# ArmingLou/seed-vc

Hardware: AMD Instinct MI355X
Metric: mel_frames_per_sec (higher is better)
Workload: dtype f16; 1 GPU; seed-uvit-tat-xlsr-tiny CFM 25 steps cfg 0.7 + HiFT, batch 64 x (P=430,S=430) per GPU; batch_per_gpu=64, global_batch=64, prompt_frames=430, diffusion_steps=25, vocoder_precision=fp16p8, lanes_per_gpu=2, parallelism=utterance-sharded x1, audio gather on rank 0

## Files before the change

seed-vc_amd/csrc/common.h:

```cpp
#pragma once
#include <atomic>
#include <hip/hip_runtime.h>
#include <stdint.h>
#include <stdio.h>
#include <string>

namespace svc {

typedef _Float16 half_t;
typedef _Float16 half8 __attribute__((ext_vector_type(8)));
typedef _Float16 half4 __attribute__((ext_vector_type(4)));
typedef _Float16 half2v __attribute__((ext_vector_type(2)));
typedef float float4v __attribute__((ext_vector_type(4)));
typedef unsigned int u32x4 __attribute__((ext_vector_type(4)));

void set_error(const std::string& msg);
const char* get_error();

#define SVC_CHECK_HIP(expr)                                                                  \
    do {                                                                                     \
        hipError_t _e = (expr);                                                              \
        if (_e != hipSuccess) {                                                              \
            svc::set_error(std::string(#expr) + ": " + hipGetErrorString(_e) + " at " + __FILE__ + \
                           ":" + std::to_string(__LINE__));                                  \
            return 1;                                                                        \
        }                                                                                    \
    } while (0)

#define SVC_REQUIRE(cond, msg)                                                               \
    do {                                                                                     \
        if (!(cond)) {                                                                       \
            svc::set_error(std::string("requirement failed: ") + #cond + " -- " + (msg));    \
            return 1;                                                                        \
        }                                                                                    \
    } while (0)

__device__ __forceinline__ float sin_sq(float x) {
    const float n = rintf(x * 0.318309886183790672f);
    float r = fmaf(n, -3.140625f, x);
    r = fmaf(n, -9.67502593994140625e-4f, r);
    r = fmaf(n, -1.509957990978376e-7f, r);
    const float r2 = r * r;
    float p = fmaf(r2, 2.6348154733568663e-06f, -0.00019822761532850564f);
    p = fmaf(p, r2, 0.008333242498338223f);
    p = fmaf(p, r2, -0.1666666567325592f);
    const float sn = fmaf(p * r2, r, r);
    return sn * sn;
}

struct DeviceState {
    int device = -1;
    void* zero_page = nullptr;
    std::atomic<unsigned long long> kconv_attr{0};
    std::atomic<bool> fused_attr{false};
};
DeviceState* device_state();
int current_device();

enum { PROF_KGEMM_F16 = 0, PROF_KGEMM_F32 = 1, PROF_ATTN = 2, PROF_FUSED = 3, PROF_N = 4 };
bool prof_enabled();
void prof_begin(int cls, hipStream_t st);
void prof_end(int cls, double flops, double bytes, hipStream_t st, unsigned long long tag = 0);

template <int MAXA, int DPT>
__device__ __forceinline__ void wait_tiles(int ahead) {
    static_assert(MAXA * DPT <= 63, "vmcnt is a 6-bit counter");
    if constexpr (MAXA <= 0) {
        asm volatile("s_waitcnt vmcnt(0)" ::: "memory");
    } else {
        if (ahead >= MAXA) asm volatile("s_waitcnt vmcnt(%0)" ::"n"(MAXA * DPT) : "memory");
        else wait_tiles<MAXA - 1, DPT>(ahead);
    }
}

__device__ __forceinline__ float act_apply(float v, int act, float slope);
__device__ __forceinline__ uint4 pack8(const float* v) {
    half8 h;
#pragma unroll
    for (int j = 0; j < 8; ++j) h[j] = (half_t)v[j];
    return *reinterpret_cast<uint4*>(&h);
}

static inline int cdiv(long a, long b) { return (int)((a + b - 1) / b); }
static inline long round_up(long a, long b) { return (a + b - 1) / b * b; }

constexpr int KG_MAX_TAPS = 48;

enum { KG_PAD_ZERO = 0, KG_PAD_REFLECT = 1, KG_PAD_CLAMP = 2 };
enum { KG_ACT_NONE = 0, KG_ACT_SILU = 1, KG_ACT_ELU = 2, KG_ACT_LRELU = 3, KG_ACT_TANH = 4, KG_ACT_ABS = 5,
       KG_ACT_CLAMP = 6 , KG_ACT_SIGMOID = 7,
       KG_ACT_GELU = 8  };
enum {
    KG_EPI_STORE = 0,
    KG_EPI_SWIGLU = 1,
    KG_EPI_TANHSIG = 2,
    KG_EPI_QKV_ROPE = 3,
    KG_EPI_STORE_GELU = 4,
};

__device__ __forceinline__ float gelu_erf(float v) { return 0.5f * v * (1.0f + erff(v * 0.70710678118654752f)); }

__device__ __forceinline__ float act_apply(float v, int act, float slope) {
    switch (act) {
        case KG_ACT_SILU: return v / (1.0f + __expf(-v));
        case KG_ACT_ELU: return v > 0.f ? v : (expm1f(v));
        case KG_ACT_LRELU: return v > 0.f ? v : v * slope;
        case KG_ACT_TANH: return tanhf(v);
        case KG_ACT_ABS: return fabsf(v);
        case KG_ACT_CLAMP: return fminf(fmaxf(v, -slope), slope);
        case KG_ACT_SIGMOID: return 1.0f / (1.0f + __expf(-v));
        default: return v;
    }
}

struct KGemmParams {
    const void* a_ptr[KG_MAX_TAPS];
    long a_ld[KG_MAX_TAPS];
    int a_shift[KG_MAX_TAPS];
    int a_ktiles[KG_MAX_TAPS];
    int n_taps;
    int Lout, a_seq_rows, a_off, a_stride, a_len, pad_mode;
    int reflect_min;
    const int* seq_len;
    const void* zero_page;
    float prof_flop_scale;
    int debug;
    int group_n;
    const void* w;
    long ldw;
    int M, N;
    int c_seq_rows, c_off;
    float* c32; long ldc32;
    half_t* c16; long ldc16;
    const float* post_a; const float* post_ib; int post_n; half_t* c16_lo;
    const float* bias;
    const float* rowvec; long ld_rowvec;
    const float* gate;   long ld_gate;
    const float* res;    long ldres;
    const float* res2;   long ldres2;
    float out_scale;
    int act; float act_slope;
    int post_relu;
    int vec_ok;
    const float* rope;
    int rope_D;
    float q_scale;
    half_t* vt; long vt_seq_stride; long vt_ld;
    int vt_mode;
};

int kgemm_launch(const KGemmParams& p, int dtype , int epi, hipStream_t st);
int kgemm_big_launch(const KGemmParams& p, int epi, hipStream_t st);

struct KConvParams {
    const void* a_hi; const void* a_lo;
// ... 87 lines not shown
```

seed-vc_amd/csrc/conv_util.h:

```cpp
#pragma once
#include <stdlib.h>
#include <string.h>

#include <string>

#include "model_util.h"

namespace svc {

struct ConvW {
    void* w = nullptr;
    float* bias = nullptr;
    long ldw = 0;
    int k = 0, cin_pad = 0, cout = 0, cout_pad = 0, dtype = 0, vd = 0;
    void* w8 = nullptr;
    long ldw8 = 0;
    int w8_exp = 0;
    int stride = 0;
};

inline int gdt(int vd) { return vd == 1 ? 1 : 0; }
inline bool is_split(int vd) { return vd == 2 || vd == 3; }
inline int cpad(int c, int vd) { return (int)round_up(c, ktile_elems(gdt(vd))); }
inline size_t vesize(int vd) { return esize(gdt(vd)); }
// ... 92 lines not shown
                } else {
                    if (pack_f16_launch(ws.v + kk, reinterpret_cast<half_t*>(out->w) + off, cin, cout, 1, (long)cout * k, k, 0, 1,
                                        out->ldw, 0, ws.scale, st)) return 1;
                }
            }
        }
        SVC_CHECK_HIP(hipMemcpyAsync(out->bias + (long)r * out->cout_pad, b->data, cout * sizeof(float),
                                     hipMemcpyDeviceToDevice, st));
    }
    return 0;
}

struct ConvRun {
    ActBuf a;
    int B = 0, Lin = 0, Lout = 0;
    int dilation = 1, stride = 1, pad_left = 0, pad_mode = KG_PAD_ZERO;
    float* c32 = nullptr; long ldc32 = 0;
    half_t* c16 = nullptr; long ldc16 = 0;
    int c_rows = 0, c_off = 0;
    const float* res = nullptr; long ldres = 0;
    const float* res2 = nullptr; long ldres2 = 0;
    float out_scale = 0.f;
    int act = KG_ACT_NONE; float act_slope = 0.f;
    int n_override = 0;
    const int* seq_len = nullptr;
    bool seq_kconv = false;
    const float* post_a = nullptr; const float* post_ib = nullptr; int post_n = 0; half_t* c16_lo = nullptr;
    int c16_lo_fmt = 0;
    bool p8 = false;
    int bm = 0;
    bool force_gemm = false;
    int* took = nullptr;
};

inline int kconv_min_n() {
    static const int v = [] { const char* e = getenv("SVC_KCONV_MIN_N"); return e ? atoi(e) : 64; }();
    return v;
}

constexpr int KCONV_MIN_ROWS = 192;

inline bool conv_p8_ok(const ConvW& w, int Lout, int dilation) {
    return w.w8 != nullptr && kconv_enabled() && (w.k - 1) * dilation <= 64 && Lout >= KCONV_MIN_ROWS && w.cout_pad >= kconv_min_n() &&
           w.cout_pad % 8 == 0;
}

inline int conv1d_run(const ConvW& w, const ConvRun& r, hipStream_t st) {
    KGemmParams p;
    memset(&p, 0, sizeof(p));
    const int nsub = is_split(w.vd) ? 3 : 1;
    SVC_REQUIRE(w.k * nsub <= KG_MAX_TAPS, "conv kernel size exceeds the tap limit");
    p.M = r.B * r.Lout;
    p.N = r.n_override ? r.n_override : w.cout_pad;
    p.Lout = r.Lout;
    p.a_seq_rows = r.Lin;
    p.a_len = r.Lin;
    p.seq_len = r.seq_len;
    p.a_stride = r.stride;
    p.pad_mode = r.pad_mode;
    p.n_taps = w.k * nsub;
    const int kt = w.cin_pad / ktile_elems(w.dtype);
    for (int t = 0; t < w.k; ++t)
        for (int sub = 0; sub < nsub; ++sub) {
            const int i = t * nsub + sub;
            p.a_ptr[i] = sub == 2 ? r.a.lo : r.a.hi;
            p.a_ld[i] = w.cin_pad;
            p.a_ktiles[i] = kt;
            p.a_shift[i] = t * r.dilation - r.pad_left;
        }
    p.w = w.w;
    p.ldw = w.ldw;
    p.bias = w.bias;
    p.c_seq_rows = r.c_rows ? r.c_rows : r.Lout;
    p.c_off = r.c_off;
    p.c32 = r.c32; p.ldc32 = r.ldc32;
    p.c16 = r.c16; p.ldc16 = r.ldc16;
    p.res = r.res; p.ldres = r.ldres;
    p.res2 = r.res2; p.ldres2 = r.ldres2;
    p.out_scale = r.out_scale;
    p.act = r.act; p.act_slope = r.act_slope;
    p.post_a = r.post_a; p.post_ib = r.post_ib; p.post_n = r.post_n; p.c16_lo = r.c16_lo;
    p.prof_flop_scale = 1.0f / nsub;
    p.vec_ok = (p.N % 8 == 0) && (r.ldc32 % 8 == 0) && (r.ldc16 % 8 == 0) && (r.ldres % 8 == 0) && (r.ldres2 % 8 == 0);
    const bool kconv_ok = !r.force_gemm && kconv_enabled() && w.dtype == 0 && r.stride == 1 && w.k >= 3 && (w.k - 1) * r.dilation <= 64 &&
                          r.pad_mode == KG_PAD_ZERO && (!r.seq_len || (r.seq_kconv && r.Lin == r.Lout)) && !r.n_override && p.vec_ok &&
                          r.Lout >= KCONV_MIN_ROWS && w.cin_pad >= 64 &&
                          p.N >= kconv_min_n();
    SVC_REQUIRE((!r.p8 && !r.c16_lo_fmt) || (kconv_ok && (!r.p8 || conv_p8_ok(w, r.Lout, r.dilation))),
                "conv1d_run: the fp8-pair operand format needs the resident-tile kernel");
    if (kconv_ok) {
        KConvParams q;
        memset(&q, 0, sizeof(q));
        q.a_hi = r.a.hi; q.a_lo = r.a.lo; q.w = r.p8 ? w.w8 : w.w; q.ldw = r.p8 ? w.ldw8 : w.ldw; q.bias = w.bias;
        q.B = r.B; q.Lin = r.Lin; q.Lout = r.Lout; q.N = p.N; q.cin_pad = w.cin_pad; q.k = w.k; q.dil = r.dilation;
        q.pad_left = r.pad_left; q.nsub = r.p8 ? 2 : nsub; q.w8_exp = w.w8_exp; q.c16_lo_fmt = r.c16_lo_fmt;
        q.c_seq_rows = p.c_seq_rows; q.c_off = p.c_off;
        q.c32 = r.c32; q.ldc32 = r.ldc32; q.c16 = r.c16; q.c16_lo = r.c16_lo; q.ldc16 = r.ldc16;
        q.post_a = r.post_a; q.post_ib = r.post_ib; q.post_n = r.post_n;
        q.res = r.res; q.ldres = r.ldres; q.res2 = r.res2; q.ldres2 = r.ldres2;
        q.out_scale = r.out_scale; q.act = r.act; q.act_slope = r.act_slope;
        q.seq_len = r.seq_len;
        q.bm = r.bm; q.took = r.took;
        return kconv_launch(q, st);
    }
    if (r.took) *r.took = 0;
    return kgemm_launch(p, w.dtype, KG_EPI_STORE, st);
}

inline int convT_run(const ConvW& w, ActBuf a, int B, int L, float* c32, int c_rows_q, int c_off_q, hipStream_t st,
                     const int* seq_len = nullptr) {
    KGemmParams p;
    memset(&p, 0, sizeof(p));
    const int nsub = is_split(w.vd) ? 3 : 1;
    p.M = B * L;
    p.N = w.stride * w.cout_pad;
    p.Lout = L;
    p.a_seq_rows = L;
    p.a_len = L;
    p.seq_len = seq_len;
    p.a_stride = 1;
    p.pad_mode = KG_PAD_ZERO;
    p.n_taps = 3 * nsub;
    const int kt = w.cin_pad / ktile_elems(w.dtype);
    for (int t = 0; t < 3; ++t)
        for (int sub = 0; sub < nsub; ++sub) {
            const int i = t * nsub + sub;
            p.a_ptr[i] = sub == 2 ? a.lo : a.hi;
            p.a_ld[i] = w.cin_pad;
            p.a_ktiles[i] = kt;
            p.a_shift[i] = t - 1;
        }
    p.w = w.w;
    p.ldw = w.ldw;
    p.bias = w.bias;
    p.c_seq_rows = c_rows_q ? c_rows_q : L;
    p.c_off = c_off_q;
    p.c32 = c32;
    p.ldc32 = p.N;
    p.vec_ok = 1;
    p.prof_flop_scale = 1.0f / nsub;
    return kgemm_launch(p, w.dtype, KG_EPI_STORE, st);
}

}
```

seed-vc_amd/csrc/fused.hip:

```cpp
#include <stdlib.h>

#include <utility>

#include "common.h"

namespace svc {

namespace {

typedef __attribute__((address_space(1))) const void* gptr_t;
typedef __attribute__((address_space(3))) void* lptr_t;

template <int D>
struct PG {
    static constexpr int NT = D / 16;
    static constexpr int KC = D / 32;
    static constexpr int SLOT_BYTES = NT * 1024;
    static constexpr int NS = D == 384 ? 5 : 4;
    static constexpr int RING = NS * SLOT_BYTES;
    static constexpr int PF = D == 384 ? 6 : 4;
    static constexpr int NVEC = 9;
    static constexpr int LDS = RING + NVEC * D * 4;
};

__device__ __forceinline__ half8 frag_read(unsigned lds_addr, int off) {
    half8 r;
    asm volatile("ds_read_b128 %0, %1 offset:%2" : "=v"(r) : "v"(lds_addr), "n"(0) : "memory");
    (void)off;
    return r;
}
template <int OFF>
__device__ __forceinline__ void frag_read_to(half8& r, unsigned lds_addr) {
    asm volatile("ds_read_b128 %0, %1 offset:%2" : "=v"(r) : "v"(lds_addr), "n"(OFF));
}
template <int N>
__device__ __forceinline__ void frag_wait(half8& r) {
    asm volatile("s_waitcnt lgkmcnt(%1)" : "+v"(r) : "n"(N));
}

template <int NF, int PF, int TM, int RFI, typename F, typename R>
__device__ __forceinline__ void stream_frags(const char* base, F&& body, R&& refill) {
    static_assert(NF * 1024 <= 65536 && PF >= 1 && PF <= 8, "ds_read offset field");
    const unsigned la = (unsigned)(uintptr_t)(lptr_t)const_cast<char*>(base);
    half8 q[PF];
    [&]<int... I>(std::integer_sequence<int, I...>) { (frag_read_to<I * 1024>(q[I], la), ...); }(std::make_integer_sequence<int, PF>{});
    [&]<int... Fi>(std::integer_sequence<int, Fi...>) {
        ([&] {
            constexpr int f = Fi;
            constexpr int pending = (NF - f < PF ? NF - f : PF) - 1;
            frag_wait<pending>(q[f % PF]);
            const half8 w = q[f % PF];
            body(f, w);
            if constexpr (f + PF < NF) frag_read_to<(f + PF) * 1024>(q[f % PF], la);
            if constexpr (f % RFI == RFI - 1) refill(f / RFI);
            __builtin_amdgcn_sched_barrier(0);
        }(), ...);
    }(std::make_integer_sequence<int, NF>{});
}

__device__ __forceinline__ void mfma_v(float4v& c, const half8 a, const half8 b) {
    asm volatile("v_mfma_f32_16x16x32_f16 %0, %1, %2, %0" : "+v"(c) : "v"(a), "v"(b));
}
__device__ __forceinline__ void mfma_guard(float4v (&a)[4][2]) {
    asm volatile("s_nop 15\n\ts_nop 3"
                 : "+v"(a[0][0]), "+v"(a[0][1]), "+v"(a[1][0]), "+v"(a[1][1]), "+v"(a[2][0]), "+v"(a[2][1]), "+v"(a[3][0]), "+v"(a[3][1]));
}
__device__ __forceinline__ void mfma_guard(float4v (&a)[4][1]) {}
template <int NF, typename F, typename R>
__device__ __forceinline__ void stream_frags_asm(const char* base, F&& body, R&& refill) {
    static_assert(NF % 4 == 0, "fragment groups of 4");
    half8 q[2][4];
#pragma unroll
    for (int i = 0; i < 4; ++i) q[0][i] = *reinterpret_cast<const half8*>(base + i * 1024);
#pragma unroll
    for (int g = 0; g < NF / 4; ++g) {
        if (g + 1 < NF / 4) {
#pragma unroll
            for (int i = 0; i < 4; ++i) q[(g + 1) & 1][i] = *reinterpret_cast<const half8*>(base + ((g + 1) * 4 + i) * 1024);
        }
        __builtin_amdgcn_sched_barrier(0);
#pragma unroll
        for (int i = 0; i < 4; ++i) body(g * 4 + i, q[g & 1][i]);
        refill(g);
        __builtin_amdgcn_sched_barrier(0);
    }
}

enum { V_AF = 0, V_BF = 1, V_GA = 2, V_GF = 3, V_AA = 4, V_BA = 5, V_BS = 6, V_AN = 7, V_BN = 8 };

template <int D, bool GATED, int TM>
__global__ __launch_bounds__(128 / (16 * TM) * 64, 128 / (16 * TM) / 4) void dit_panel_kernel(const PanelParams p) {
    using G = PG<D>;
    constexpr int NT = G::NT, KC = G::KC, NS = G::NS, PF = G::PF;
    constexpr int NW = 128 / (16 * TM), NTHR = NW * 64, DPS = NT / NW, RFI = NT / DPS;
    constexpr bool ASM_SIDE = D == 512 && TM == 2;
    extern __shared__ __attribute__((aligned(16))) char smem[];
    float* vec = reinterpret_cast<float*>(smem + G::RING);

    const int tid = threadIdx.x, lane = tid & 63;
    const int wave = __builtin_amdgcn_readfirstlane(tid >> 6);
    const int fr = lane & 15, fq = lane >> 4;
    const int m0 = blockIdx.x * 128 + wave * (16 * TM);

    for (int c = tid; c < D; c += NTHR) {
        const float one = p.add_one ? 1.f : 0.f;
        vec[V_AF * D + c] = p.g_ffn ? p.g_ffn[c] * (p.w_f ? one + p.w_f[c] : 1.f) : 0.f;
        vec[V_BF * D + c] = p.b_f ? p.b_f[c] : 0.f;
        vec[V_GA * D + c] = p.gate_a ? p.gate_a[c] : 1.f;
        vec[V_GF * D + c] = p.gate_f ? p.gate_f[c] : 1.f;
        vec[V_AA * D + c] = p.g_attn ? p.g_attn[c] * (p.w_a ? one + p.w_a[c] : 1.f) : 0.f;
        vec[V_BA * D + c] = p.b_a ? p.b_a[c] : 0.f;
        vec[V_BS * D + c] = p.bskip ? p.bskip[c] : 0.f;
        vec[V_AN * D + c] = p.g_fin ? p.g_fin[c] * (p.w_fin ? one + p.w_fin[c] : 1.f) : 0.f;
        vec[V_BN * D + c] = p.b_fin ? p.b_fin[c] : 0.f;
    }
    __syncthreads();

    const char* wsrc = reinterpret_cast<const char*>(p.wstream) + wave * (G::SLOT_BYTES / NW) + lane * 16;
    int s_next = 0, stage = 0, fill = NS - 1, s_issued = 0;
    auto piece = [&](const char* src, char* dst, int i) {
// ... 508 lines not shown
```

seed-vc_amd/csrc/kconv.hip:

```cpp
#include <math.h>
#include <stdlib.h>
#include <string.h>

#include "common.h"

namespace svc {

namespace {

constexpr int CB_NW = 8, CB_NT = CB_NW * 64;
constexpr int CB_SPAN = 64;
constexpr int cb_a_bytes(int bm) { return (bm + CB_SPAN) * 128; }
constexpr int CB_EPI_LD = 68;
constexpr int cb_ns(int bn, int bm) { return bm == 128 ? 2 : (bm < 256 ? 3 : (bn == 128 ? 5 : 8)); }
constexpr int cb_lds(int bn, int bm) { return 2 * cb_a_bytes(bm) + cb_ns(bn, bm) * bn * 128; }

__device__ __forceinline__ int cswz(int row) { return row & 7; }

template <int NSUB, int BN, int BM, bool RAGGED>
__global__ __launch_bounds__(CB_NT, BM < 256 ? 2 : 1) void kconv_kernel(const KConvParams p) {
    constexpr int CB_N = BN, CB_M = BM;
    constexpr int CB_NS = cb_ns(BN, BM);
    constexpr int CB_A_BYTES = cb_a_bytes(BM);
    constexpr int CB_W_BYTES = BN * 128;
    constexpr int WROWS_M = BN == 128 ? BM / 4 : BM / 8;
    constexpr int TM = WROWS_M / 16;
    static_assert(TM >= 1, "tile");
    constexpr int WDPT = BN / 64;
    extern __shared__ __attribute__((aligned(16))) char smem[];
    char* a_hi = smem;
    char* a_lo = smem + CB_A_BYTES;
    char* w_ring = smem + 2 * CB_A_BYTES;

    const int tid = threadIdx.x, lane = tid & 63, wave = tid >> 6;
    const int wave_u = __builtin_amdgcn_readfirstlane(wave);
    const int n_mt = (p.Lout + CB_M - 1) / CB_M;
    const int n_nt = (p.N + CB_N - 1) / CB_N;
    const int nblk = gridDim.x;
    const int xq = nblk >> 3, xr = nblk & 7, xcd = blockIdx.x & 7;
    const int bid = (xcd < xr ? xcd * (xq + 1) : xr * (xq + 1) + (xcd - xr) * xq) + (blockIdx.x >> 3);
    const int tile_n = bid % n_nt;
    const int rest = bid / n_nt;
    const int tile_m = rest % n_mt;
    const int b = rest / n_mt;
    const int p0 = tile_m * CB_M;
    int lin = p.Lin;
    if constexpr (RAGGED) {
        lin = p.seq_len[b];
        if (p0 >= lin) return;
    }
    const int n0 = tile_n * CB_N;
    const int span = (p.k - 1) * p.dil;
    const int R = CB_M + span;
    const int nchunks = p.cin_pad / 64;
    const int total = nchunks * p.k * NSUB;

    typedef __attribute__((address_space(1))) const void* gptr_t;
    typedef __attribute__((address_space(3))) void* lptr_t;
    const char* zero_ = reinterpret_cast<const char*>(p.zero_page);

    const int wm0 = BN == 128 ? (wave >> 1) * WROWS_M : wave * WROWS_M, wn0 = BN == 128 ? (wave & 1) * 64 : 0;
    const int fr = lane & 15, fq = lane >> 4;
    float4v acc[TM][4];
#pragma unroll
    for (int i = 0; i < TM; ++i)
#pragma unroll
        for (int j = 0; j < 4; ++j) acc[i][j] = (float4v){0.f, 0.f, 0.f, 0.f};

    const int c8 = tid & 7, rr = tid >> 3;
    const half_t* wrow[WDPT];
#pragma unroll
    for (int i = 0; i < WDPT; ++i) {
        const int row = rr + 64 * i;
        wrow[i] = reinterpret_cast<const half_t*>(p.w) + (long)(n0 + row) * p.ldw + ((c8 ^ cswz(row)) << 3);
    }
    auto issue_w = [&](int it, int stage) {
        const int c = it / (p.k * NSUB);
        const int ts = it - c * (p.k * NSUB);
        const long col = (long)ts * p.cin_pad + 64L * c;
        char* dst = w_ring + stage * CB_W_BYTES + wave_u * 1024;
#pragma unroll
        for (int i = 0; i < WDPT; ++i)
            __builtin_amdgcn_global_load_lds((gptr_t)(wrow[i] + col), (lptr_t)(dst + i * 64 * 128), 16, 0, 0);
    };
    auto issue_a = [&](int c) {
        for (int i = 0; i * 64 < R; ++i) {
            const int row = rr + 64 * i;
            const int pos = p0 - p.pad_left + row;
            const bool ok = (row < R) & (pos >= 0) & (pos < lin);
            const long off = (((long)b * p.Lin + (ok ? pos : 0)) * p.cin_pad + 64L * c + ((c8 ^ cswz(row)) << 3)) * 2;
            const char* sh = ok ? reinterpret_cast<const char*>(p.a_hi) + off : zero_;
            __builtin_amdgcn_global_load_lds((gptr_t)sh, (lptr_t)(a_hi + (64 * i + wave_u * 8) * 128), 16, 0, 0);
            if constexpr (NSUB != 1) {
                const char* sl = ok ? reinterpret_cast<const char*>(p.a_lo) + off : zero_;
                __builtin_amdgcn_global_load_lds((gptr_t)sl, (lptr_t)(a_lo + (64 * i + wave_u * 8) * 128), 16, 0, 0);
            }
        }
    };

#pragma unroll
    for (int s_ = 0; s_ < CB_NS - 1; ++s_)
        if (s_ < total) issue_w(s_, s_);
    int stage = 0, fill = CB_NS - 1, it = 0;
    for (int c = 0; c < nchunks; ++c) {
        asm volatile("s_waitcnt vmcnt(0)" ::: "memory");
        asm volatile("s_barrier" ::: "memory");
        issue_a(c);
        asm volatile("s_waitcnt vmcnt(0)" ::: "memory");
        asm volatile("s_barrier" ::: "memory");
        for (int t = 0; t < p.k; ++t) {
            const int shift = t * p.dil;
#pragma unroll
            for (int s = 0; s < NSUB; ++s, ++it) {
                const int ahead = total - 1 - it;
                wait_tiles<CB_NS - 2, WDPT>(ahead);
                asm volatile("s_barrier" ::: "memory");
                if (it + CB_NS - 1 < total) issue_w(it + CB_NS - 1, fill);
                const char* at = ((NSUB == 3 && s == 2) || (NSUB == 2 && s == 1)) ? a_lo : a_hi;
                const char* wt = w_ring + stage * CB_W_BYTES;
                if constexpr (NSUB == 2) {
                    if (s == 1) {
                        typedef int v8i __attribute__((ext_vector_type(8)));
                        v8i af8[TM], bf8[4];
#pragma unroll
                        for (int mt = 0; mt < TM; ++mt) {
                            const int row = wm0 + mt * 16 + fr + shift;
                            const u32x4 x0 = *reinterpret_cast<const u32x4*>(at + row * 128 + ((fq ^ cswz(row)) << 4));
                            const u32x4 x1 = *reinterpret_cast<const u32x4*>(at + row * 128 + (((4 + fq) ^ cswz(row)) << 4));
                            af8[mt] = (v8i){(int)x0[0], (int)x0[1], (int)x0[2], (int)x0[3], (int)x1[0], (int)x1[1], (int)x1[2], (int)x1[3]};
                        }
#pragma unroll
                        for (int nt = 0; nt < 4; ++nt) {
                            const int row = wn0 + nt * 16 + fr;
                            const u32x4 x0 = *reinterpret_cast<const u32x4*>(wt + row * 128 + ((fq ^ cswz(row)) << 4));
                            const u32x4 x1 = *reinterpret_cast<const u32x4*>(wt + row * 128 + (((4 + fq) ^ cswz(row)) << 4));
                            bf8[nt] = (v8i){(int)x0[0], (int)x0[1], (int)x0[2], (int)x0[3], (int)x1[0], (int)x1[1], (int)x1[2], (int)x1[3]};
                        }
                        const int sc_a = 127 - 11, sc_b = 127 - p.w8_exp;
#pragma unroll
                        for (int mt = 0; mt < TM; ++mt)
#pragma unroll
                            for (int nt = 0; nt < 4; ++nt)
                                acc[mt][nt] = __builtin_amdgcn_mfma_scale_f32_16x16x128_f8f6f4(af8[mt], bf8[nt], acc[mt][nt], 0, 0, 0, sc_a, 0, sc_b);
                        stage = stage + 1 == CB_NS ? 0 : stage + 1;
                        fill = fill + 1 == CB_NS ? 0 : fill + 1;
                        continue;
                    }
                }
#pragma unroll
                for (int ks = 0; ks < 2; ++ks) {
                    u32x4 af[TM], bf[4];
                    const int chunk = ks * 4 + fq;
#pragma unroll
                    for (int mt = 0; mt < TM; ++mt) {
                        const int row = wm0 + mt * 16 + fr + shift;
                        af[mt] = *reinterpret_cast<const u32x4*>(at + row * 128 + ((chunk ^ cswz(row)) << 4));
                    }
#pragma unroll
                    for (int nt = 0; nt < 4; ++nt) {
                        const int row = wn0 + nt * 16 + fr;
                        bf[nt] = *reinterpret_cast<const u32x4*>(wt + row * 128 + ((chunk ^ cswz(row)) << 4));
                    }
#pragma unroll
                    for (int mt = 0; mt < TM; ++mt)
#pragma unroll
                        for (int nt = 0; nt < 4; ++nt)
                            acc[mt][nt] = __builtin_amdgcn_mfma_f32_16x16x32_f16(__builtin_bit_cast(half8, af[mt]),
                                                                                 __builtin_bit_cast(half8, bf[nt]), acc[mt][nt], 0, 0, 0);
                }
                stage = stage + 1 == CB_NS ? 0 : stage + 1;
                fill = fill + 1 == CB_NS ? 0 : fill + 1;
            }
        }
    }
    asm volatile("s_waitcnt vmcnt(0)" ::: "memory");
    __syncthreads();

    constexpr int RP = TM >= 2 ? 32 : 16;
    float* ep = reinterpret_cast<float*>(smem) + wave * RP * CB_EPI_LD;
#pragma unroll
    for (int pass = 0; pass < TM * 16 / RP; ++pass) {
        if (pass > 0) __syncthreads();
#pragma unroll
        for (int mi = 0; mi < RP / 16; ++mi)
#pragma unroll
            for (int nt = 0; nt < 4; ++nt)
#pragma unroll
                for (int r = 0; r < 4; ++r)
                    ep[(mi * 16 + fq * 4 + r) * CB_EPI_LD + nt * 16 + fr] = acc[pass * (RP / 16) + mi][nt][r];
        __syncthreads();
#pragma unroll
        for (int i = 0; i < RP / 8; ++i) {
            const int ch = lane + 64 * i;
            const int row = ch >> 3, cc = ch & 7;
            const int pos = p0 + wm0 + pass * RP + row;
            const int n = n0 + wn0 + cc * 8;
            float v[8];
            {
                const float4v x0 = *reinterpret_cast<const float4v*>(ep + row * CB_EPI_LD + cc * 8);
                const float4v x1 = *reinterpret_cast<const float4v*>(ep + row * CB_EPI_LD + cc * 8 + 4);
#pragma unroll
                for (int j = 0; j < 4; ++j) { v[j] = x0[j]; v[4 + j] = x1[j]; }
            }
            if (pos >= p.Lout || n >= p.N) continue;
            const long orow = (long)b * p.c_seq_rows + p.c_off + pos;
            if (p.bias) {
                const float4v b0 = *reinterpret_cast<const float4v*>(p.bias + n);
                const float4v b1 = *reinterpret_cast<const float4v*>(p.bias + n + 4);
#pragma unroll
                for (int j = 0; j < 4; ++j) { v[j] += b0[j]; v[4 + j] += b1[j]; }
            }
            if (p.act != KG_ACT_NONE) {
#pragma unroll
                for (int j = 0; j < 8; ++j) v[j] = act_apply(v[j], p.act, p.act_slope);
            }
            if (p.res) {
                const float4v q0 = *reinterpret_cast<const float4v*>(p.res + orow * p.ldres + n);
                const float4v q1 = *reinterpret_cast<const float4v*>(p.res + orow * p.ldres + n + 4);
#pragma unroll
                for (int j = 0; j < 4; ++j) { v[j] += q0[j]; v[4 + j] += q1[j]; }
            }
            if (p.out_scale != 0.f) {
#pragma unroll
                for (int j = 0; j < 8; ++j) v[j] *= p.out_scale;
            }
            if (p.res2) {
                const float4v q0 = *reinterpret_cast<const float4v*>(p.res2 + orow * p.ldres2 + n);
                const float4v q1 = *reinterpret_cast<const float4v*>(p.res2 + orow * p.ldres2 + n + 4);
#pragma unroll
                for (int j = 0; j < 4; ++j) { v[j] += q0[j]; v[4 + j] += q1[j]; }
            }
            if (p.c32) {
                *reinterpret_cast<float4v*>(p.c32 + orow * p.ldc32 + n) = (float4v){v[0], v[1], v[2], v[3]};
                *reinterpret_cast<float4v*>(p.c32 + orow * p.ldc32 + n + 4) = (float4v){v[4], v[5], v[6], v[7]};
            }
            if (p.post_a) {
                float lo[8];
                float hf[8];
#pragma unroll
                for (int j = 0; j < 8; ++j) {
                    const int nn = n + j;
                    const float sv = nn < p.post_n ? v[j] + p.post_ib[nn] * sin_sq(p.post_a[nn] * v[j]) : 0.f;
                    const half_t hh = (half_t)sv;
                    v[j] = sv;
                    lo[j] = sv - (float)hh;
                    hf[j] = (float)hh;
                }
                if (p.c16_lo) {
                    if (p.c16_lo_fmt) {
                                const u32x4 pr = {lo_pair_p8(hf[0], lo[0]) | (lo_pair_p8(hf[1], lo[1]) << 16), lo_pair_p8(hf[2], lo[2]) | (lo_pair_p8(hf[3], lo[3]) << 16),
                                                  lo_pair_p8(hf[4], lo[4]) | (lo_pair_p8(hf[5], lo[5]) << 16), lo_pair_p8(hf[6], lo[6]) | (lo_pair_p8(hf[7], lo[7]) << 16)};
                                *reinterpret_cast<u32x4*>(p.c16_lo + orow * p.ldc16 + n) = pr;
                            }
                    else *reinterpret_cast<uint4*>(p.c16_lo + orow * p.ldc16 + n) = pack8(lo);
                }
            }
            if (p.c16) *reinterpret_cast<uint4*>(p.c16 + orow * p.ldc16 + n) = pack8(v);
        }
    }
}


__global__ void absmax_kernel(const float* __restrict__ src, int n0, int n1, int n2, long s0, long s1, long s2,
                              const float* __restrict__ scale, float* __restrict__ out) {
    __shared__ float red[256];
    float m = 0.f;
    const long total = (long)n0 * n1 * n2;
    for (long i = (long)blockIdx.x * 256 + threadIdx.x; i < total; i += 256L * gridDim.x) {
        const int i2 = (int)(i % n2);
        const long r = i / n2;
        const int i1 = (int)(r % n1), i0 = (int)(r / n1);
        float v = src[i0 * s0 + i1 * s1 + i2 * s2];
        if (scale) v *= scale[i0];
        m = fmaxf(m, fabsf(v));
    }
    red[threadIdx.x] = m;
    __syncthreads();
    for (int o = 128; o > 0; o >>= 1) {
        if ((int)threadIdx.x < o) red[threadIdx.x] = fmaxf(red[threadIdx.x], red[threadIdx.x + o]);
        __syncthreads();
    }
    if (threadIdx.x == 0) atomicMax(reinterpret_cast<unsigned*>(out), __float_as_uint(red[0]));
}

__global__ void pack_p8_kernel(const float* __restrict__ src, unsigned short* __restrict__ dst, int n0, int n1, int n2, long s0, long s1,
                               long s2, long d0, long d1, long d2, const float* __restrict__ scale, float sw) {
    const long i = (long)blockIdx.x * blockDim.x + threadIdx.x;
    const long total = (long)n0 * n1 * n2;
    if (i >= total) return;
    const int i2 = (int)(i % n2);
    const long r = i / n2;
    const int i1 = (int)(r % n1), i0 = (int)(r / n1);
    float v = src[i0 * s0 + i1 * s1 + i2 * s2];
    if (scale) v *= scale[i0];
    const float hi = (float)(half_t)v, lo = v - hi;
    const float b0 = fminf(fmaxf(lo * sw * 2048.f, -448.f), 448.f), b1 = fminf(fmaxf(hi * sw, -448.f), 448.f);
    dst[i0 * d0 + i1 * d1 + i2 * d2] = (unsigned short)((unsigned)__builtin_amdgcn_cvt_pk_fp8_f32(b0, b1, 0, false) & 0xffffu);
}

}

int kconv_pack_p8(const float* src, unsigned short* dst, int n0, int n1, int n2, long s0, long s1, long s2, long d0, long d1, long d2,
                  const float* scale, int* exp_out, hipStream_t st) {
    float* d_max = nullptr;
    SVC_CHECK_HIP(hipMalloc(&d_max, sizeof(float)));
    SVC_CHECK_HIP(hipMemsetAsync(d_max, 0, sizeof(float), st));
    hipLaunchKernelGGL(absmax_kernel, dim3(256), dim3(256), 0, st, src, n0, n1, n2, s0, s1, s2, scale, d_max);
    float mx = 0.f;
    hipError_t e = hipMemcpyAsync(&mx, d_max, sizeof(float), hipMemcpyDeviceToHost, st);
    if (e == hipSuccess) e = hipStreamSynchronize(st);
    (void)hipFree(d_max);
    SVC_CHECK_HIP(e);
    int ex = 0;
    if (mx > 0.f) {
        ex = (int)floorf(log2f(224.0f / mx));
        ex = ex > 24 ? 24 : (ex < -24 ? -24 : ex);
    }
    *exp_out = ex;
    const long n = (long)n0 * n1 * n2;
    hipLaunchKernelGGL(pack_p8_kernel, dim3(cdiv(n, 256)), dim3(256), 0, st, src, dst, n0, n1, n2, s0, s1, s2, d0, d1, d2, scale,
                       ldexpf(1.0f, ex));
    SVC_CHECK_HIP(hipGetLastError());
    return 0;
}

namespace {
}

bool kconv_enabled() {
    static const bool off = [] { const char* e = getenv("SVC_KCONV"); return e && e[0] == '0'; }();
    return !off;
}

template <int NSUB, int BN, int BM, bool RAGGED>
int kconv_go(DeviceState* ds, const KConvParams& p, int grid, hipStream_t st) {
    constexpr unsigned long long bit = 1ull << ((NSUB == 3 ? 1 : (NSUB == 2 ? 2 : 0)) + 3 * ((BN == 64 ? 3 : 0) + (BM == 64 ? 0 : (BM == 128 ? 1 : 2))) +
                                                (RAGGED ? 18 : 0));
    if (!(ds->kconv_attr.load(std::memory_order_acquire) & bit)) {
        SVC_CHECK_HIP(hipFuncSetAttribute(reinterpret_cast<const void*>(kconv_kernel<NSUB, BN, BM, RAGGED>), hipFuncAttributeMaxDynamicSharedMemorySize,
                                          cb_lds(BN, BM)));
        ds->kconv_attr.fetch_or(bit, std::memory_order_release);
    }
    hipLaunchKernelGGL((kconv_kernel<NSUB, BN, BM, RAGGED>), dim3(grid), dim3(CB_NT), cb_lds(BN, BM), st, p);
    SVC_CHECK_HIP(hipGetLastError());
    return 0;
}

int kconv_launch(const KConvParams& p_in, hipStream_t st) {
    SVC_REQUIRE(p_in.k >= 1 && (p_in.k - 1) * p_in.dil <= CB_SPAN && p_in.cin_pad % 64 == 0 && p_in.N % 8 == 0, "kconv shape");
    SVC_REQUIRE(!p_in.seq_len || p_in.Lin == p_in.Lout, "kconv: per-sequence lengths need Lin == Lout");
    SVC_REQUIRE(p_in.act != KG_ACT_GELU, "kconv: KG_ACT_GELU exists in the tap-GEMM's STORE epilogue only");
    DeviceState* ds = device_state();
    if (!ds) return 1;
    KConvParams p = p_in;
    p.zero_page = ds->zero_page;
    const int bn = p.N <= 64 ? 64 : 128;
    static const int bm_env = [] { const char* e = getenv("SVC_KCONV_BM"); return e ? atoi(e) : 0; }();
    const long g256 = (long)p.B * cdiv(p.Lout, 256) * cdiv(p.N, bn);
    int bm = 256;
    if (bn == 128) bm = g256 <= 96 ? 64 : 128;
    if (bn == 128 && (bm_env == 64 || bm_env == 128 || bm_env == 256)) bm = bm_env;
    if (bn == 128 && (p.bm == 64 || p.bm == 128 || p.bm == 256)) bm = p.bm;
    if (p.took) *p.took = 1 | (bm << 8) | (bn << 20);
    const int grid = p.B * cdiv(p.Lout, bm) * cdiv(p.N, bn);
    if (grid <= 0) return 0;
    const bool prof = prof_enabled();
    if (prof) prof_begin(PROF_KGEMM_F16, st);
    int rc;
#define SVC_KCONV_GO_(BN_, BM_, RG_) (p.nsub == 3 ? kconv_go<3, BN_, BM_, RG_>(ds, p, grid, st) : (p.nsub == 2 ? kconv_go<2, BN_, BM_, RG_>(ds, p, grid, st) : kconv_go<1, BN_, BM_, RG_>(ds, p, grid, st)))
#define SVC_KCONV_GO(BN_, BM_) (p.seq_len ? SVC_KCONV_GO_(BN_, BM_, true) : SVC_KCONV_GO_(BN_, BM_, false))
    if (bn == 128) {
        if (bm == 64) rc = SVC_KCONV_GO(128, 64);
        else if (bm == 128) rc = SVC_KCONV_GO(128, 128);
        else rc = SVC_KCONV_GO(128, 256);
    } else {
        rc = SVC_KCONV_GO(64, 256);
    }
#undef SVC_KCONV_GO
#undef SVC_KCONV_GO_
    if (rc) return rc;
    if (prof) {
        const double M = (double)p.B * p.Lout, K = (double)p.k * p.cin_pad;
        double bytes = (M * p.cin_pad * (p.nsub != 1 ? 2 : 1) + (double)p.N * K * p.nsub) * 2.0;
        bytes += M * p.N * ((p.c32 ? 4 : 0) + (p.c16 ? 2 : 0) + (p.c16_lo ? 2 : 0) + (p.res ? 4 : 0) + (p.res2 ? 4 : 0));
        const unsigned long long tag = ((unsigned long long)(long)M << 40) | ((unsigned long long)(p.N & 0xFFFFF) << 20) |
                                       ((unsigned long long)((long)(K * p.nsub) & 0xFFFF) << 4) | 4u;
        prof_end(PROF_KGEMM_F16, 2.0 * M * p.N * K, bytes, st, tag);
    }
    return 0;
}

}
```

Baseline: 137,100 mel-frames/s.

## Add software-pipelined kconv main loop with double-buffered LDS fragments and interleaved refills

Adds a PIPE variant of the resident-tile conv kernel. It double-buffers A/B fragment reads from LDS across MFMA groups, interleaves the global-to-LDS weight refills between MFMA instructions, and uses explicit lgkmcnt waits and sched barriers, with higher occupancy launch bounds (4 for BM<256). The variant is enabled by default and can be turned off with SVC_KCONV_PIPE=0. It also lets kconv handle k<3 convs when a bm is explicitly requested. The aim is to hide LDS and global latency behind MFMA work, at the risk of register pressure from the tighter launch bounds and more complex scheduling.

```diff
diff --git a/seed-vc_amd/csrc/common.h b/seed-vc_amd/csrc/common.h
--- a/seed-vc_amd/csrc/common.h
+++ b/seed-vc_amd/csrc/common.h
@@ -52,6 +52,7 @@
     int device = -1;
     void* zero_page = nullptr;
     std::atomic<unsigned long long> kconv_attr{0};
+    std::atomic<unsigned long long> kconv_pipe_attr{0};
     std::atomic<bool> fused_attr{false};
 };
 DeviceState* device_state();
@@ -71,6 +72,20 @@
         if (ahead >= MAXA) asm volatile("s_waitcnt vmcnt(%0)" ::"n"(MAXA * DPT) : "memory");
         else wait_tiles<MAXA - 1, DPT>(ahead);
     }
+}
+
+template <int OFF, typename V>
+__device__ __forceinline__ void frag_read_to(V& r, unsigned lds_addr) {
+    static_assert(sizeof(V) == 16 && OFF >= 0 && OFF < 65536, "ds_read_b128 offset field");
+    asm volatile("ds_read_b128 %0, %1 offset:%2" : "=v"(r) : "v"(lds_addr), "n"(OFF));
+}
+template <int N, typename V>
+__device__ __forceinline__ void frag_wait(V& r) {
+    asm volatile("s_waitcnt lgkmcnt(%1)" : "+v"(r) : "n"(N));
+}
+template <typename V>
+__device__ __forceinline__ void frag_pin(V& r) {
+    asm volatile("" : "+v"(r));
 }
 
 __device__ __forceinline__ float act_apply(float v, int act, float slope);
diff --git a/seed-vc_amd/csrc/conv_util.h b/seed-vc_amd/csrc/conv_util.h
--- a/seed-vc_amd/csrc/conv_util.h
+++ b/seed-vc_amd/csrc/conv_util.h
@@ -198,7 +198,7 @@
     p.post_a = r.post_a; p.post_ib = r.post_ib; p.post_n = r.post_n; p.c16_lo = r.c16_lo;
     p.prof_flop_scale = 1.0f / nsub;
     p.vec_ok = (p.N % 8 == 0) && (r.ldc32 % 8 == 0) && (r.ldc16 % 8 == 0) && (r.ldres % 8 == 0) && (r.ldres2 % 8 == 0);
-    const bool kconv_ok = !r.force_gemm && kconv_enabled() && w.dtype == 0 && r.stride == 1 && w.k >= 3 && (w.k - 1) * r.dilation <= 64 &&
+    const bool kconv_ok = !r.force_gemm && kconv_enabled() && w.dtype == 0 && r.stride == 1 && (w.k >= 3 || r.bm != 0) && (w.k - 1) * r.dilation <= 64 &&
                           r.pad_mode == KG_PAD_ZERO && (!r.seq_len || (r.seq_kconv && r.Lin == r.Lout)) && !r.n_override && p.vec_ok &&
                           r.Lout >= KCONV_MIN_ROWS && w.cin_pad >= 64 &&
                           p.N >= kconv_min_n();
diff --git a/seed-vc_amd/csrc/fused.hip b/seed-vc_amd/csrc/fused.hip
--- a/seed-vc_amd/csrc/fused.hip
+++ b/seed-vc_amd/csrc/fused.hip
@@ -28,14 +28,6 @@
     asm volatile("ds_read_b128 %0, %1 offset:%2" : "=v"(r) : "v"(lds_addr), "n"(0) : "memory");
     (void)off;
     return r;
-}
-template <int OFF>
-__device__ __forceinline__ void frag_read_to(half8& r, unsigned lds_addr) {
-    asm volatile("ds_read_b128 %0, %1 offset:%2" : "=v"(r) : "v"(lds_addr), "n"(OFF));
-}
-template <int N>
-__device__ __forceinline__ void frag_wait(half8& r) {
-    asm volatile("s_waitcnt lgkmcnt(%1)" : "+v"(r) : "n"(N));
 }
 
 template <int NF, int PF, int TM, int RFI, typename F, typename R>
diff --git a/seed-vc_amd/csrc/kconv.hip b/seed-vc_amd/csrc/kconv.hip
--- a/seed-vc_amd/csrc/kconv.hip
+++ b/seed-vc_amd/csrc/kconv.hip
@@ -1,6 +1,8 @@
 #include <math.h>
 #include <stdlib.h>
 #include <string.h>
+#include <type_traits>
+#include <utility>
 
 #include "common.h"
 
@@ -17,8 +19,25 @@
 
 __device__ __forceinline__ int cswz(int row) { return row & 7; }
 
-template <int NSUB, int BN, int BM, bool RAGGED>
-__global__ __launch_bounds__(CB_NT, BM < 256 ? 2 : 1) void kconv_kernel(const KConvParams p) {
+template <int OFF, int STRIDE, typename V, size_t... I>
+__device__ __forceinline__ void frag_read_seq(V* r, unsigned addr, std::index_sequence<I...>) {
+    (frag_read_to<OFF + (int)I * STRIDE>(r[I], addr), ...);
+}
+template <int OFF, int STRIDE, int N, typename V>
+__device__ __forceinline__ void frag_read_n(V* r, unsigned addr) {
+    frag_read_seq<OFF, STRIDE>(r, addr, std::make_index_sequence<N>{});
+}
+template <typename F, size_t... I>
+__device__ __forceinline__ void static_for_seq(F&& f, std::index_sequence<I...>) {
+    (f(std::integral_constant<int, (int)I>{}), ...);
+}
+template <int N, typename F>
+__device__ __forceinline__ void static_for(F&& f) {
+    static_for_seq(f, std::make_index_sequence<N>{});
+}
+
+template <int NSUB, int BN, int BM, bool RAGGED, bool PIPE>
+__global__ __launch_bounds__(CB_NT, BM < 256 ? (PIPE ? 4 : 2) : 1) void kconv_kernel(const KConvParams p) {
     constexpr int CB_N = BN, CB_M = BM;
     constexpr int CB_NS = cb_ns(BN, BM);
     constexpr int CB_A_BYTES = cb_a_bytes(BM);
@@ -32,7 +51,8 @@
     char* a_lo = smem + CB_A_BYTES;
     char* w_ring = smem + 2 * CB_A_BYTES;
 
-    const int tid = threadIdx.x, lane = tid & 63, wave = tid >> 6;
+    const int tid = threadIdx.x;
+    int lane = tid & 63, wave = tid >> 6;
     const int wave_u = __builtin_amdgcn_readfirstlane(wave);
     const int n_mt = (p.Lout + CB_M - 1) / CB_M;
     const int n_nt = (p.N + CB_N - 1) / CB_N;
@@ -59,8 +79,8 @@
     typedef __attribute__((address_space(3))) void* lptr_t;
     const char* zero_ = reinterpret_cast<const char*>(p.zero_page);
 
-    const int wm0 = BN == 128 ? (wave >> 1) * WROWS_M : wave * WROWS_M, wn0 = BN == 128 ? (wave & 1) * 64 : 0;
-    const int fr = lane & 15, fq = lane >> 4;
+    int wm0 = BN == 128 ? (wave >> 1) * WROWS_M : wave * WROWS_M, wn0 = BN == 128 ? (wave & 1) * 64 : 0;
+    int fr = lane & 15, fq = lane >> 4;
     float4v acc[TM][4];
 #pragma unroll
     for (int i = 0; i < TM; ++i)
@@ -98,6 +118,186 @@
         }
     };
 
+    if constexpr (PIPE) {
+    constexpr bool P8 = NSUB == 2;
+    typedef int v8i __attribute__((ext_vector_type(8)));
+    const unsigned lds0 = (unsigned)(uintptr_t)(lptr_t)smem;
+    const unsigned wrd = lds0 + 2 * CB_A_BYTES + (wn0 + fr) * 128;
+    const unsigned wo0 = wrd + ((fq ^ cswz(fr)) << 4), wo1 = wrd + (((4 + fq) ^ cswz(fr)) << 4);
+    u32x4 fa0[TM], fb0[4], fa1[TM], fb1[4];
+    u32x4 pa0[TM], pa1[TM];
+    const int sc_a = 127 - 11, sc_b = 127 - p.w8_exp;
+    auto a_addr = [&](int shift, unsigned& a0, unsigned& a1) {
+        const int row = wm0 + fr + shift;
+        const unsigned base = lds0 + row * 128;
+        a0 = base + ((fq ^ cswz(row)) << 4);
+        a1 = base + (((4 + fq) ^ cswz(row)) << 4);
+    };
+    auto rd_a0 = [&](auto sic, unsigned a0, unsigned a1) {
+        constexpr int S = decltype(sic)::value;
+        constexpr int LO = ((NSUB == 3 && S == 2) || (P8 && S == 1)) ? CB_A_BYTES : 0;
+        if constexpr (P8 && S == 1) {
+            frag_read_n<LO, 2048, TM>(pa0, a0);
+            frag_read_n<LO, 2048, TM>(pa1, a1);
+        } else {
+            frag_read_n<LO, 2048, TM>(fa0, a0);
+        }
+    };
+    auto rd_b0 = [&](auto sic, unsigned w0, unsigned w1) {
+        constexpr int S = decltype(sic)::value;
+        if constexpr (P8 && S == 1) {
+            frag_read_n<0, 2048, 2>(fb0, w0);
+            frag_read_n<0, 2048, 2>(fb0 + 2, w1);
+        } else {
+            frag_read_n<0, 2048, 4>(fb0, w0);
+        }
+    };
+    auto rd_g1 = [&](auto sic, unsigned a1, unsigned w0, unsigned w1) {
+        constexpr int S = decltype(sic)::value;
+        constexpr int LO = (NSUB == 3 && S == 2) ? CB_A_BYTES : 0;
+        if constexpr (P8 && S == 1) {
+            frag_read_n<4096, 2048, 2>(fb1, w0);
+            frag_read_n<4096, 2048, 2>(fb1 + 2, w1);
+        } else {
+            frag_read_n<LO, 2048, TM>(fa1, a1);
+            frag_read_n<0, 2048, 4>(fb1, w1);
+        }
+    };
+    auto wait_g0 = [&](auto sic, auto pend) {
+        constexpr int S = decltype(sic)::value;
+        frag_wait<decltype(pend)::value>(fb0[3]);
+#pragma unroll
+        for (int i = 0; i < 3; ++i) frag_pin(fb0[i]);
+#pragma unroll
+        for (int i = 0; i < TM; ++i) {
+            if constexpr (P8 && S == 1) { frag_pin(pa0[i]); frag_pin(pa1[i]); }
+            else frag_pin(fa0[i]);
+        }
+    };
+    auto wait_g1 = [&](auto sic, auto pend) {
+        constexpr int S = decltype(sic)::value;
+        frag_wait<decltype(pend)::value>(fb1[3]);
+#pragma unroll
+        for (int i = 0; i < 3; ++i) frag_pin(fb1[i]);
+        if constexpr (!(P8 && S == 1)) {
+#pragma unroll
+            for (int i = 0; i < TM; ++i) frag_pin(fa1[i]);
+        }
+    };
+    auto cat8 = [](const u32x4 x0, const u32x4 x1) {
+        return (v8i){(int)x0[0], (int)x0[1], (int)x0[2], (int)x0[3], (int)x1[0], (int)x1[1], (int)x1[2], (int)x1[3]};
+    };
+    auto mfma_g0 = [&](auto sic) {
+        constexpr int S = decltype(sic)::value;
+        if constexpr (P8 && S == 1) {
+#pragma unroll
+            for (int mt = 0; mt < TM; ++mt)
+#pragma unroll
+                for (int nt = 0; nt < 2; ++nt)
+                    acc[mt][nt] = __builtin_amdgcn_mfma_scale_f32_16x16x128_f8f6f4(cat8(pa0[mt], pa1[mt]), cat8(fb0[nt], fb0[2 + nt]), acc[mt][nt],
+                                                                                   0, 0, 0, sc_a, 0, sc_b);
+        } else {
+#pragma unroll
+            for (int mt = 0; mt < TM; ++mt)
+#pragma unroll
+                for (int nt = 0; nt < 4; ++nt)
+                    acc[mt][nt] = __builtin_amdgcn_mfma_f32_16x16x32_f16(__builtin_bit_cast(half8, fa0[mt]), __builtin_bit_cast(half8, fb0[nt]),
+                                                                         acc[mt][nt], 0, 0, 0);
+        }
+#pragma unroll
+        for (int mt = 0; mt < TM; ++mt)
+#pragma unroll
+            for (int nt = 0; nt < ((P8 && S == 1) ? 2 : 4); ++nt) frag_pin(acc[mt][nt]);
+    };
+    int rf_c = 0, rf_ts = CB_NS;
+    while (rf_ts >= p.k * NSUB) { rf_ts -= p.k * NSUB; ++rf_c; }
+    auto mfma_g1 = [&](auto sic, bool rf, int stage) {
+        constexpr int S = decltype(sic)::value;
+        constexpr int NPM = (P8 && S == 1) ? 2 : 4, NM = TM * NPM;
+        static_assert(NM >= WDPT, "refill instructions");
+        const int col = rf_ts * p.cin_pad + 64 * rf_c;
+        char* dst = w_ring + stage * CB_W_BYTES + wave_u * 1024;
+        static_for<NM>([&](auto jc) {
+            constexpr int j = decltype(jc)::value;
+            if constexpr (P8 && S == 1) {
+                constexpr int mt = j / 2, nt = j % 2;
+                acc[mt][2 + nt] = __builtin_amdgcn_mfma_scale_f32_16x16x128_f8f6f4(cat8(pa0[mt], pa1[mt]), cat8(fb1[nt], fb1[2 + nt]), acc[mt][2 + nt],
+                                                                                   0, 0, 0, sc_a, 0, sc_b);
+            } else {
+                constexpr int mt = j / 4, nt = j % 4;
+                acc[mt][nt] = __builtin_amdgcn_mfma_f32_16x16x32_f16(__builtin_bit_cast(half8, fa1[mt]), __builtin_bit_cast(half8, fb1[nt]),
+                                                                     acc[mt][nt], 0, 0, 0);
+            }
+            if constexpr (j < WDPT) {
+                frag_pin(acc[j / NPM][(P8 && S == 1 ? 2 : 0) + j % NPM]);
+                __builtin_amdgcn_sched_barrier(0);
+                if (rf) __builtin_amdgcn_global_load_lds((gptr_t)(wrow[j] + col), (lptr_t)(dst + j * 64 * 128), 16, 0, 0);
+                __builtin_amdgcn_sched_barrier(0);
+            }
+        });
+#pragma unroll
+        for (int mt = 0; mt < TM; ++mt)
+#pragma unroll
+            for (int nt = (P8 && S == 1) ? 2 : 0; nt < 4; ++nt) frag_pin(acc[mt][nt]);
+        if (rf && ++rf_ts == p.k * NSUB) { rf_ts = 0; ++rf_c; }
+    };
+
+#pragma unroll
+    for (int s_ = 0; s_ < CB_NS; ++s_)
+        if (s_ < total) issue_w(s_, s_);
+    int stage = 0, it = 0;
+    for (int c = 0; c < nchunks; ++c) {
+        asm volatile("s_waitcnt vmcnt(0)" ::: "memory");
+        asm volatile("s_barrier" ::: "memory");
+        issue_a(c);
+        asm volatile("s_waitcnt vmcnt(0)" ::: "memory");
+        asm volatile("s_barrier" ::: "memory");
+        unsigned ca0, ca1;
+        a_addr(0, ca0, ca1);
+        rd_a0(std::integral_constant<int, 0>{}, ca0, ca1);
+        rd_b0(std::integral_constant<int, 0>{}, wo0 + stage * CB_W_BYTES, wo1 + stage * CB_W_BYTES);
+        __builtin_amdgcn_sched_barrier(0);
+        for (int t = 0; t < p.k; ++t) {
+            const bool last_t = t + 1 == p.k;
+            static_for<NSUB>([&](auto sic) {
+                constexpr int S = decltype(sic)::value;
+                constexpr int SN = S + 1 < NSUB ? S + 1 : 0;
+                constexpr bool PN = P8 && SN == 1;
+                constexpr int N_G1 = (P8 && S == 1) ? 4 : TM + 4;
+                constexpr int N_A0 = PN ? 2 * TM : TM;
+                const std::integral_constant<int, SN> snc{};
+                const bool pf = S + 1 < NSUB || !last_t;
+                const bool more = it + 1 < total;
+                const int nx = stage + 1 == CB_NS ? 0 : stage + 1;
+                const unsigned ws = stage * CB_W_BYTES, wn = nx * CB_W_BYTES;
+                rd_g1(sic, ca1, wo0 + ws, wo1 + ws);
+                if constexpr (S + 1 == NSUB) a_addr((t + 1) * p.dil, ca0, ca1);
+                __builtin_amdgcn_sched_barrier(0);
+                wait_g0(sic, std::integral_constant<int, N_G1>{});
+                __builtin_amdgcn_sched_barrier(0);
+                mfma_g0(sic);
+                __builtin_amdgcn_sched_barrier(0);
+                if (pf) {
+                    rd_a0(snc, ca0, ca1);
+                    wait_g1(sic, std::integral_constant<int, N_A0>{});
+                } else {
+                    wait_g1(sic, std::integral_constant<int, 0>{});
+                }
+                __builtin_amdgcn_sched_barrier(0);
+                if (more) {
+                    wait_tiles<CB_NS - 2, WDPT>(total - 2 - it);
+                    asm volatile("s_barrier" ::: "memory");
+                }
+                if (pf) rd_b0(snc, wo0 + wn, wo1 + wn);
+                __builtin_amdgcn_sched_barrier(0);
+                mfma_g1(sic, it + CB_NS < total, stage);
+                __builtin_amdgcn_sched_barrier(0);
+                stage = nx;
+                ++it;
+            });
+        }
+    }
+    } else {
 #pragma unroll
     for (int s_ = 0; s_ < CB_NS - 1; ++s_)
         if (s_ < total) issue_w(s_, s_);
@@ -172,6 +372,14 @@
                 fill = fill + 1 == CB_NS ? 0 : fill + 1;
             }
         }
+    }
+    }
+    if constexpr (PIPE) {
+        int t2 = tid;
+        asm volatile("" : "+v"(t2));
+        lane = t2 & 63, wave = t2 >> 6;
+        wm0 = BN == 128 ? (wave >> 1) * WROWS_M : wave * WROWS_M, wn0 = BN == 128 ? (wave & 1) * 64 : 0;
+        fr = lane & 15, fq = lane >> 4;
     }
     asm volatile("s_waitcnt vmcnt(0)" ::: "memory");
     __syncthreads();
@@ -332,16 +540,17 @@
     return !off;
 }
 
-template <int NSUB, int BN, int BM, bool RAGGED>
+template <int NSUB, int BN, int BM, bool RAGGED, bool PIPE>
 int kconv_go(DeviceState* ds, const KConvParams& p, int grid, hipStream_t st) {
     constexpr unsigned long long bit = 1ull << ((NSUB == 3 ? 1 : (NSUB == 2 ? 2 : 0)) + 3 * ((BN == 64 ? 3 : 0) + (BM == 64 ? 0 : (BM == 128 ? 1 : 2))) +
                                                 (RAGGED ? 18 : 0));
-    if (!(ds->kconv_attr.load(std::memory_order_acquire) & bit)) {
-        SVC_CHECK_HIP(hipFuncSetAttribute(reinterpret_cast<const void*>(kconv_kernel<NSUB, BN, BM, RAGGED>), hipFuncAttributeMaxDynamicSharedMemorySize,
-                                          cb_lds(BN, BM)));
-        ds->kconv_attr.fetch_or(bit, std::memory_order_release);
-    }
-    hipLaunchKernelGGL((kconv_kernel<NSUB, BN, BM, RAGGED>), dim3(grid), dim3(CB_NT), cb_lds(BN, BM), st, p);
+    std::atomic<unsigned long long>& attr = PIPE ? ds->kconv_pipe_attr : ds->kconv_attr;
+    if (!(attr.load(std::memory_order_acquire) & bit)) {
+        SVC_CHECK_HIP(hipFuncSetAttribute(reinterpret_cast<const void*>(kconv_kernel<NSUB, BN, BM, RAGGED, PIPE>),
+                                          hipFuncAttributeMaxDynamicSharedMemorySize, cb_lds(BN, BM)));
+        attr.fetch_or(bit, std::memory_order_release);
+    }
+    hipLaunchKernelGGL((kconv_kernel<NSUB, BN, BM, RAGGED, PIPE>), dim3(grid), dim3(CB_NT), cb_lds(BN, BM), st, p);
     SVC_CHECK_HIP(hipGetLastError());
     return 0;
 }
@@ -364,10 +573,13 @@
     if (p.took) *p.took = 1 | (bm << 8) | (bn << 20);
     const int grid = p.B * cdiv(p.Lout, bm) * cdiv(p.N, bn);
     if (grid <= 0) return 0;
+    const char* pipe_env = getenv("SVC_KCONV_PIPE");
+    const bool pipe = !(pipe_env && pipe_env[0] == '0' && pipe_env[1] == 0);
     const bool prof = prof_enabled();
     if (prof) prof_begin(PROF_KGEMM_F16, st);
     int rc;
-#define SVC_KCONV_GO_(BN_, BM_, RG_) (p.nsub == 3 ? kconv_go<3, BN_, BM_, RG_>(ds, p, grid, st) : (p.nsub == 2 ? kconv_go<2, BN_, BM_, RG_>(ds, p, grid, st) : kconv_go<1, BN_, BM_, RG_>(ds, p, grid, st)))
+#define SVC_KCONV_GO__(BN_, BM_, RG_, PP_) (p.nsub == 3 ? kconv_go<3, BN_, BM_, RG_, PP_>(ds, p, grid, st) : (p.nsub == 2 ? kconv_go<2, BN_, BM_, RG_, PP_>(ds, p, grid, st) : kconv_go<1, BN_, BM_, RG_, PP_>(ds, p, grid, st)))
+#define SVC_KCONV_GO_(BN_, BM_, RG_) (pipe ? SVC_KCONV_GO__(BN_, BM_, RG_, true) : SVC_KCONV_GO__(BN_, BM_, RG_, false))
 #define SVC_KCONV_GO(BN_, BM_) (p.seq_len ? SVC_KCONV_GO_(BN_, BM_, true) : SVC_KCONV_GO_(BN_, BM_, false))
     if (bn == 128) {
         if (bm == 64) rc = SVC_KCONV_GO(128, 64);
@@ -378,6 +590,7 @@
     }
 #undef SVC_KCONV_GO
 #undef SVC_KCONV_GO_
+#undef SVC_KCONV_GO__
     if (rc) return rc;
     if (prof) {
         const double M = (double)p.B * p.Lout, K = (double)p.k * p.cin_pad;
```

Result: no change. 137,900 mel-frames/s (median of 6 runs) (+0.6%).
